# W-Ted/F3D-Gaus

Hardware: AMD Instinct MI355X
Metric: rendered views/sec at 256x256 (N Gaussians, K cams) (higher is better)
Workload: dtype f32; 1 GPU; C2: 1 image/GPU, 196608 Gaussians (sigma0=0.01), 120-view orbit @256x256, GOF forward raster only; timed region = render + 8-bit RGB frames copied to pinned host memory; compositing arithmetic: fast = error-free float32 pairs for the float64 island + hardware exp/rcp/rsq; every channel within 1e-4 of the oracle (RGB <= 3e-7), EXCEPT that the distortion channel (values 1e-7..1e-5 from cancelling fl; gaussians=196608, views=120, resolution=256, tile_cull=1, views_per_call=120, render_mode=fast, channels=all, parallelism=single GPU

## Files before the change

f3d-gaus_amd/csrc/f3dg_api.hip:

```cpp
#include "f3dg_common.h"

#include <stdio.h>
#include <string.h>
#include <time.h>
#include <mutex>
#include <vector>

namespace {

thread_local char g_last_error[512] = "";

size_t align_up(size_t x, size_t a) { return (x + a - 1) / a * a; }

__global__ void init_header_kernel(F3dgHeader* hdr, unsigned capacity, unsigned alpha_fast = 0, unsigned save_aux = 0)
{
    if (threadIdx.x < 64) {
        unsigned* w = reinterpret_cast<unsigned*>(hdr);
        w[threadIdx.x] = 0;
    }
    __syncthreads();
    if (threadIdx.x == 0) { hdr->capacity = capacity; hdr->alpha_fast = alpha_fast; hdr->save_aux = save_aux; }
}

__global__ void fill_background_kernel(int V, size_t HW, const float* __restrict__ bg, int bg_per_view,
// ... 175 lines not shown
    }
    g_prof.bwd.clear();
    if (h_calls) *h_calls = (int)g_prof.calls.size();
    g_prof.calls.clear();
    if (h_stage_ms) {
        for (int i = 0; i < ST_COUNT; i++) h_stage_ms[i] = sum[i];
        for (int i = 0; i < BW_COUNT; i++) h_stage_ms[ST_COUNT + i] = bsum[i];
    }
    return F3DG_OK;
}

int f3dg_set_hip_error(hipError_t e, const char* where)
{
    snprintf(g_last_error, sizeof g_last_error, "%s: %s", where, hipGetErrorString(e));
    return F3DG_ERR_HIP;
}

extern "C" const char* f3dg_version(void) { return "f3dg-hip gfx950 0.2.0"; }
extern "C" const char* f3dg_last_error(void) { return g_last_error; }

int f3dg_sort_passes(int V, int T);

F3dgLayout f3dg_layout(int P, int W, int H, int V, long long cap)
{
    F3dgLayout L;
    memset(&L, 0, sizeof L);
    const size_t VP = (size_t)V * (size_t)(P > 0 ? P : 1);
    const size_t HW = (size_t)W * H;
    const size_t T = (size_t)((W + F3DG_TILE - 1) / F3DG_TILE) * ((H + F3DG_TILE - 1) / F3DG_TILE);
    const size_t C = (size_t)(cap > 0 ? cap : 1);
    L.sort_blocks = (unsigned)((C + F3DG_SORT_CHUNK - 1) / F3DG_SORT_CHUNK);
    const size_t scan_a = (VP + F3DG_SCAN_CHUNK - 1) / F3DG_SCAN_CHUNK;
    const size_t gsort_blocks = (size_t)V * (((size_t)(P > 0 ? P : 1) + F3DG_SORT_CHUNK - 1) / F3DG_SORT_CHUNK);
    const size_t tile_blocks = (size_t)L.sort_blocks + (size_t)V;
    const size_t hist_blocks = gsort_blocks > tile_blocks ? gsort_blocks : tile_blocks;
    const size_t scan_b = ((size_t)256 * hist_blocks + F3DG_SCAN_CHUNK - 1) / F3DG_SCAN_CHUNK;
    L.scan_tmp_elems = (unsigned)((scan_a > scan_b ? scan_a : scan_b) + 1);

    size_t off = 0;
    auto take = [&](size_t bytes) { size_t o = off; off = align_up(off + bytes, 256); return o; };
    L.header = take(sizeof(F3dgHeader));
    L.rec = take(VP * sizeof(F3dgRec));
    L.means2D = take(VP * sizeof(float2));
    L.bbox = take(VP * sizeof(float4));
    L.cull = take(VP * sizeof(float4));
    L.depths = take(VP * sizeof(float));
    L.conic = take(VP * sizeof(float4));
    L.radii = take(VP * sizeof(int));
    L.tiles = take(VP * sizeof(unsigned));
    L.offsets = take(VP * sizeof(unsigned));
    L.clamped = take(VP);
    L.rects = take(VP * sizeof(uint2));
    L.gsort = take(4 * VP * sizeof(unsigned));
    L.scan_tmp = take((size_t)L.scan_tmp_elems * sizeof(unsigned));
    L.keys[0] = take(C * 8);
    L.keys[1] = take(C * 4);
    L.vals[0] = take(C * 4);
    L.vals[1] = take(C * 4);
    L.segtab_minmax = (unsigned)((size_t)2 * (V + 1) + (size_t)8 * (V / 8 + 2));
    L.segtab = take(((size_t)L.segtab_minmax + (size_t)2 * V + 2 * gsort_blocks) * sizeof(unsigned));
    L.hist = take((size_t)256 * hist_blocks * sizeof(unsigned));
    L.ranges = take((size_t)V * T * sizeof(uint2));
    L.final_T = take((size_t)V * 4 * HW * sizeof(float));
    L.n_contrib = take((size_t)V * 2 * HW * sizeof(unsigned));
    L.bwd_acc = take(VP * 16 * sizeof(double));
    L.small_cap = f3dg_small_shape(P, W, H, V) ? (unsigned)F3DG_SMALL_CAP : 0u;
    L.small_boxes = take(L.small_cap ? (size_t)V * ((P + 63) / 64) * sizeof(uint2) : 0);
    L.small_cnt = take((size_t)V * T * sizeof(unsigned));
// ... 446 lines not shown
```

f3d-gaus_amd/csrc/f3dg_binning.hip:

```cpp
#include "f3dg_common.h"

namespace {

typedef unsigned long long u64;
typedef unsigned int u32;

__global__ void __launch_bounds__(F3DG_BLOCK)
scan_reduce_kernel(const u32* __restrict__ in, u64 n, u32* __restrict__ block_sums)
{
    __shared__ u32 wsum[F3DG_BLOCK / 64];
    const u64 base = (u64)blockIdx.x * F3DG_SCAN_CHUNK;
    u32 s = 0;
#pragma unroll
    for (int i = 0; i < F3DG_SCAN_ITEMS; i++) {
        const u64 k = base + (u64)i * F3DG_BLOCK + threadIdx.x;
        if (k < n) s += in[k];
    }
#pragma unroll
    for (int off = 32; off > 0; off >>= 1) s += __shfl_down(s, off, 64);
    if ((threadIdx.x & 63) == 0) wsum[threadIdx.x >> 6] = s;
    __syncthreads();
    if (threadIdx.x == 0) block_sums[blockIdx.x] = wsum[0] + wsum[1] + wsum[2] + wsum[3];
}

// ... 140 lines not shown
                const u32 key = (u32)w[q];
                atomicAdd(&hw[digit(key)], 1u);
                if (MINMAX && key != 0xFFFFFFFFu) { kmin = key < kmin ? key : kmin; kmax = key > kmax ? key : kmax; }
            }
        }
    }
    __shared__ u32 wmm[2][F3DG_BLOCK / 64];
    if (MINMAX) {
#pragma unroll
        for (int off = 32; off > 0; off >>= 1) {
            const u32 a = __shfl_down(kmin, off, 64), b = __shfl_down(kmax, off, 64);
            kmin = a < kmin ? a : kmin; kmax = b > kmax ? b : kmax;
        }
        if ((threadIdx.x & 63) == 0) { wmm[0][threadIdx.x >> 6] = kmin; wmm[1][threadIdx.x >> 6] = kmax; }
    }
    __syncthreads();
    if (MINMAX && threadIdx.x == 0) {
        u32 a = wmm[0][0], b = wmm[1][0];
#pragma unroll
        for (int w = 1; w < F3DG_BLOCK / 64; w++) { a = wmm[0][w] < a ? wmm[0][w] : a; b = wmm[1][w] > b ? wmm[1][w] : b; }
        minmax[0] = a; minmax[1] = b;
    }
    hist[ck.obase + (u64)threadIdx.x * ck.cps + ck.c] = h[0][threadIdx.x] + h[1][threadIdx.x] + h[2][threadIdx.x] + h[3][threadIdx.x];
}

struct ScatterShared {
    u32 cnt[F3DG_BLOCK / 64][256];
    u32 lbase[256];
    u32 gdelta[256];
    u32 wtot[F3DG_BLOCK / 64];
    u32 sval[F3DG_SORT_CHUNK];
};

template <typename K, bool IOTA, typename DIGIT>
__device__ __forceinline__ void scatter_chunk(const K* __restrict__ keys_in, const u32* __restrict__ vals_in, K* __restrict__ keys_out,
                                              u32* __restrict__ vals_out, const SegChunk& ck, const DIGIT digit,
                                              const u32* __restrict__ offsets , ScatterShared& sh, K* skey)
{
    const u32 n = ck.n;
    const u64 block_base = (u64)ck.c * F3DG_SORT_CHUNK;
    const u32 in_block = (u32)((n - block_base) < (u64)F3DG_SORT_CHUNK ? (n - block_base) : (u64)F3DG_SORT_CHUNK);
    const int lane = threadIdx.x & 63, wave = threadIdx.x >> 6;
#pragma unroll
    for (int w = 0; w < F3DG_BLOCK / 64; w++) sh.cnt[w][threadIdx.x] = 0;
    __syncthreads();

    const u64 wave_base = block_base + (u64)wave * (64 * F3DG_SORT_ITEMS);
    u32 key[F3DG_SORT_ITEMS];
    u32 val[F3DG_SORT_ITEMS];
    u32 rank[F3DG_SORT_ITEMS];
    const u64 lane_lt = ((u64)1 << lane) - 1;
#pragma unroll
    for (int r = 0; r < F3DG_SORT_ITEMS; r++) {
        const u64 i = wave_base + (u64)r * 64 + lane;
        const bool valid = i < n;
        key[r] = valid ? (u32)keys_in[ck.seg_base + i] : 0u;
        val[r] = IOTA ? (u32)i : (valid ? vals_in[ck.seg_base + i] : 0u);
    }
#pragma unroll
    for (int r = 0; r < F3DG_SORT_ITEMS; r++) {
        const u64 i = wave_base + (u64)r * 64 + lane;
        const bool valid = i < n;
        const u32 d = digit(key[r]);
        u64 diff = 0;
#pragma unroll
        for (int b = 0; b < 8; b++) {
            const u32 own = (u32)((int)(d << (31 - b)) >> 31);
            const u64 bal = __ballot(own != 0u);
            diff |= bal ^ (((u64)own << 32) | own);
        }
        const u64 same = __ballot(valid) & ~diff;
        const u32 below = (u32)__popcll(same & lane_lt);
        const u32 prev = sh.cnt[wave][d];
        rank[r] = prev + below;
        __builtin_amdgcn_wave_barrier();
        if (valid && below == 0) sh.cnt[wave][d] = prev + (u32)__popcll(same);
        __builtin_amdgcn_wave_barrier();
    }
    __syncthreads();
    {
        const u32 d = threadIdx.x;
        const u32 c0 = sh.cnt[0][d], c1 = sh.cnt[1][d], c2 = sh.cnt[2][d], c3 = sh.cnt[3][d];
        const u32 tot = c0 + c1 + c2 + c3;
        u32 x = tot;
#pragma unroll
        for (int off = 1; off < 64; off <<= 1) {
            const u32 y = __shfl_up(x, off, 64);
            if (lane >= off) x += y;
        }
        if (lane == 63) sh.wtot[wave] = x;
        __syncthreads();
        u32 excl = x - tot;
        for (int w = 0; w < wave; w++) excl += sh.wtot[w];
        sh.lbase[d] = excl;
        sh.gdelta[d] = offsets[ck.obase + (u64)d * ck.cps + ck.c] - excl;
        sh.cnt[0][d] = excl;
        sh.cnt[1][d] = excl + c0;
        sh.cnt[2][d] = excl + c0 + c1;
        sh.cnt[3][d] = excl + c0 + c1 + c2;
    }
    __syncthreads();
#pragma unroll
    for (int r = 0; r < F3DG_SORT_ITEMS; r++) {
        const u64 i = wave_base + (u64)r * 64 + lane;
        if (i < n) {
            const u32 d = digit(key[r]);
            const u32 slot = sh.cnt[wave][d] + rank[r];
            skey[slot] = (K)key[r];
            sh.sval[slot] = val[r];
        }
    }
    __syncthreads();
    for (u32 slot = threadIdx.x; slot < in_block; slot += F3DG_BLOCK) {
        const K k = skey[slot];
        const u32 d = digit((u32)k);
        const u32 pos = sh.gdelta[d] + slot;
        if (keys_out) keys_out[pos] = k;
        vals_out[pos] = sh.sval[slot];
    }
}

__device__ __forceinline__ SegChunk fixed_chunk(u32 seg_len, u32 cps)
{
    u32 seg, c;
    f3dg_xcd_map(blockIdx.x, gridDim.x / cps, cps, seg, c);
    SegChunk ck;
    ck.seg_base = (u64)seg * seg_len; ck.obase = (u64)seg * 256u * cps; ck.n = seg_len; ck.cps = cps; ck.c = c; ck.seg = seg;
    return ck;
}

__device__ __forceinline__ bool gsort_compact(const u32* __restrict__ minmax, u32 view, u32& kbase)
{
    const u32 kmin = minmax[2 * view], kmax = minmax[2 * view + 1];
    kbase = kmin & 0xFFFF0000u;
    return kmin <= kmax && ((kmax - kbase) >> 24) == 0u;
}

template <int PASS>
__global__ void __launch_bounds__(F3DG_BLOCK)
gsort_hist_kernel(const u32* __restrict__ keys, u32 seg_len, u32 cps, u32* __restrict__ hist, const u32* __restrict__ minmax,
                  u32* __restrict__ chunk_minmax)
{
    __shared__ u32 h[F3DG_BLOCK / 64][256];
    const SegChunk ck = fixed_chunk(seg_len, cps);
    if constexpr (PASS == 0) {
        hist_chunk<u32, ShiftDigit>(keys, ck, ShiftDigit{0}, hist, h);
    } else if constexpr (PASS == 1) {
        hist_chunk<u32, ShiftDigit, true>(keys, ck, ShiftDigit{8}, hist, h, chunk_minmax + 2 * ((size_t)ck.seg * cps + ck.c));
    } else {
        u32 kbase;
        const bool compact = gsort_compact(minmax, ck.seg, kbase);
        if (!compact) {
// ... 49 lines not shown
        kmin = a < kmin ? a : kmin; kmax = b > kmax ? b : kmax;
    }
#pragma unroll
    for (int off = 32; off > 0; off >>= 1) {
        const u32 a = __shfl_down(kmin, off, 64), b = __shfl_down(kmax, off, 64);
        kmin = a < kmin ? a : kmin; kmax = b > kmax ? b : kmax;
    }
    if (threadIdx.x == 0) { minmax[2 * blockIdx.x] = kmin; minmax[2 * blockIdx.x + 1] = kmax; }
}

template <int PASS>
__global__ void __launch_bounds__(F3DG_BLOCK)
gsort_scatter_kernel(const u32* __restrict__ keys_in, const u32* __restrict__ vals_in, u32* __restrict__ keys_out,
                     u32* __restrict__ vals_out, u32 seg_len, u32 cps, const u32* __restrict__ offsets, const u32* __restrict__ minmax)
{
    __shared__ ScatterShared sh;
    __shared__ u32 skey[F3DG_SORT_CHUNK];
    const SegChunk ck = fixed_chunk(seg_len, cps);
    if constexpr (PASS == 0) {
        scatter_chunk<u32, true, ShiftDigit>(keys_in, vals_in, keys_out, vals_out, ck, ShiftDigit{0}, offsets, sh, skey);
    } else if constexpr (PASS == 1) {
        scatter_chunk<u32, false, ShiftDigit>(keys_in, vals_in, keys_out, vals_out, ck, ShiftDigit{8}, offsets, sh, skey);
    } else {
        u32 kbase;
        const bool compact = gsort_compact(minmax, ck.seg, kbase);
        if (!compact)
            scatter_chunk<u32, false, ShiftDigit>(keys_in, vals_in, PASS == 3 ? (u32*)nullptr : keys_out, vals_out, ck, ShiftDigit{8 * PASS}, offsets, sh, skey);
        else if constexpr (PASS == 2)
            scatter_chunk<u32, false, CompactDigit>(keys_in, vals_in, (u32*)nullptr, vals_out, ck, CompactDigit{kbase}, offsets, sh, skey);
    }
}

__global__ void __launch_bounds__(512)
view_segments_kernel(int V, int P, const u32* __restrict__ offsets_sorted, const F3dgHeader* __restrict__ hdr, u32* __restrict__ vstart,
                     u32* __restrict__ bglob, u32* __restrict__ xprefix, u32 xstride)
{
    __shared__ u32 carry;
    __shared__ u32 wtot[8];
    const u32 lane = threadIdx.x & 63u, wave = threadIdx.x >> 6;
    const bool dead = hdr->overflow != 0;
    auto start_of = [&](u32 v) -> u32 {
        const u64 i = (u64)v * (u64)P;
        return (dead || i == 0) ? 0u : offsets_sorted[i - 1];
    };
    auto chunks_of = [&](u32 v) -> u32 {
        const u32 n = start_of(v + 1) - start_of(v);
        return (n + F3DG_SORT_CHUNK - 1) / F3DG_SORT_CHUNK;
    };
    if (threadIdx.x == 0) carry = 0;
    __syncthreads();
    for (u32 v0 = 0; v0 < (u32)V; v0 += 512) {
        const u32 v = v0 + threadIdx.x;
        const u32 c = v < (u32)V ? chunks_of(v) : 0u;
        u32 x = c;
#pragma unroll
        for (int off = 1; off < 64; off <<= 1) {
            const u32 y = __shfl_up(x, off, 64);
            if (lane >= (u32)off) x += y;
        }
        if (lane == 63) wtot[wave] = x;
        __syncthreads();
        u32 woff = carry;
        for (u32 w = 0; w < wave; w++) woff += wtot[w];
        if (v < (u32)V) { vstart[v] = start_of(v); bglob[v] = woff + x - c; }
        __syncthreads();
        if (threadIdx.x == 511) carry = woff + x;
        __syncthreads();
    }
    if (threadIdx.x == 0) { vstart[V] = start_of((u32)V); bglob[V] = carry; }
    const u32 nk = ((u32)V > wave) ? ((u32)V - wave + 7u) / 8u : 0u;
    u32 run = 0;
    for (u32 k0 = 0; k0 < nk; k0 += 64) {
        const u32 k = k0 + lane;
        const u32 c = k < nk ? chunks_of(wave + 8u * k) : 0u;
        u32 x = c;
#pragma unroll
        for (int off = 1; off < 64; off <<= 1) {
            const u32 y = __shfl_up(x, off, 64);
            if (lane >= (u32)off) x += y;
        }
        if (k < nk) xprefix[wave * xstride + k] = run + x - c;
        run += __shfl(x, 63, 64);
    }
    if (lane == 0) xprefix[wave * xstride + nk] = run;
}

__global__ void __launch_bounds__(F3DG_BLOCK)
ranges_from_offsets_kernel(u32 V, u32 T, int tile_bits, const u32* __restrict__ bglob, const u32* __restrict__ offsets,
                           const F3dgHeader* __restrict__ hdr, uint2* __restrict__ ranges)
{
    const u32 i = blockIdx.x * F3DG_BLOCK + threadIdx.x;
    if (i >= V * T) return;
    const u32 v = i / T, t = i % T;
    const u32 b0 = bglob[v], cpv = bglob[v + 1] - b0;
    uint2 r = make_uint2(0u, 0u);
    if (cpv != 0u && !hdr->overflow) {
        const u32 d = ((v << tile_bits) | t) & 255u;
        const u32 lo = offsets[256ull * b0 + (u64)d * cpv], hi = offsets[256ull * b0 + (u64)(d + 1u) * cpv];
        if (hi > lo) r = make_uint2(lo, hi);
    }
    ranges[i] = r;
}

__device__ __forceinline__ bool var_chunk(const SegTable& st, u32 f, u32& k, SegChunk& ck)
{
    const u32 x = blockIdx.x & 7u;
    const u32* xp = st.xprefix + x * st.xstride;
    const u32 nk = (st.V > x) ? (st.V - x + 7u) / 8u : 0u;
    while (k < nk && f >= xp[k + 1]) k++;
    if (k >= nk) return false;
    const u32 v = x + 8u * k;
    const u32 s0 = st.vstart[v], b0 = st.bglob[v];
    ck.seg_base = s0; ck.n = st.vstart[v + 1] - s0; ck.cps = st.bglob[v + 1] - b0; ck.obase = 256ull * b0; ck.c = f - xp[k];
    return true;
}

template <typename K>
__global__ void __launch_bounds__(F3DG_BLOCK)
radix2_hist_var_kernel(const K* __restrict__ keys, SegTable st, int shift, u32 mask, u32* __restrict__ hist)
{
    __shared__ u32 h[F3DG_BLOCK / 64][256];
    u32 k = 0;
    SegChunk ck;
    for (u32 f = blockIdx.x >> 3; var_chunk(st, f, k, ck); f += gridDim.x >> 3)
        hist_chunk<K, ShiftDigit>(keys, ck, ShiftDigit{shift, mask}, hist, h);
}

template <typename K>
__global__ void __launch_bounds__(F3DG_BLOCK)
radix2_scatter_var_kernel(const K* __restrict__ keys_in, const u32* __restrict__ vals_in, K* __restrict__ keys_out,
                          u32* __restrict__ vals_out, SegTable st, int shift, u32 mask, const u32* __restrict__ offsets)
{
    __shared__ ScatterShared sh;
    __shared__ K skey[F3DG_SORT_CHUNK];
    u32 k = 0;
    SegChunk ck;
    for (u32 f = blockIdx.x >> 3; var_chunk(st, f, k, ck); f += gridDim.x >> 3) {
        scatter_chunk<K, false, ShiftDigit>(keys_in, vals_in, keys_out, vals_out, ck, ShiftDigit{shift, mask}, offsets, sh, skey);
        __syncthreads();
    }
}

__global__ void __launch_bounds__(F3DG_BLOCK)
gsort_gather_rects_kernel(int P, u32* __restrict__ gv0, u32* __restrict__ gv1, const u32* __restrict__ minmax,
                          const uint2* __restrict__ rects, u32* __restrict__ tiles_sorted, u32* __restrict__ rx)
{
    constexpr int ITEMS = 4;
    unsigned view, chunk;
    const unsigned cpv = (unsigned)((P + F3DG_BLOCK * ITEMS - 1) / (F3DG_BLOCK * ITEMS));
    f3dg_xcd_map(blockIdx.x, gridDim.x / cpv, cpv, view, chunk);
    const size_t vb = (size_t)view * P;
    u32 kbase;
    const bool pass2 = gsort_compact(minmax, view, kbase);
    const u32* perm = pass2 ? gv1 : gv0;
    u32* ry = pass2 ? gv0 : gv1;
    const int k0 = (int)(chunk * F3DG_BLOCK * ITEMS + threadIdx.x);
    u32 id[ITEMS];
    uint2 r[ITEMS];
#pragma unroll
    for (int i = 0; i < ITEMS; i++) { const int k = k0 + i * F3DG_BLOCK; id[i] = k < P ? perm[vb + k] : 0u; }
#pragma unroll
    for (int i = 0; i < ITEMS; i++) { const int k = k0 + i * F3DG_BLOCK; r[i] = k < P ? rects[vb + id[i]] : make_uint2(0u, 0u); }
#pragma unroll
    for (int i = 0; i < ITEMS; i++) {
        const int k = k0 + i * F3DG_BLOCK;
        if (k < P) {
            tiles_sorted[vb + k] = (((r[i].x >> 16) & F3DG_RECT_COORD) - (r[i].x & F3DG_RECT_COORD)) *
                                   (((r[i].y >> 16) & F3DG_RECT_COORD) - (r[i].y & F3DG_RECT_COORD));
            rx[vb + k] = r[i].x;
            ry[vb + k] = r[i].y;
        }
    }
}

#define F3DG_DUP_CAP 3072
template <typename G>
__global__ void __launch_bounds__(F3DG_BLOCK)
duplicate_sorted_kernel(int P, int tile_bits, int grid_x, const u32* __restrict__ gv0, const u32* __restrict__ gv1,
                        const u32* __restrict__ minmax, const u32* __restrict__ rx,
                        const u32* __restrict__ offsets_sorted,
                        const F3dgHeader* __restrict__ hdr, G* __restrict__ kgrp, u32* __restrict__ vals)
{
    __shared__ G sk[F3DG_DUP_CAP];
    __shared__ u32 sv[F3DG_DUP_CAP];
    if (hdr->overflow) return;
    const int k = blockIdx.x * F3DG_BLOCK + threadIdx.x;
    const int v = blockIdx.y;
    u32 kbase;
    const bool pass2 = gsort_compact(minmax, (u32)v, kbase);
    const u32* perm = pass2 ? gv1 : gv0;
    const u32* ry = pass2 ? gv0 : gv1;
    const size_t first = (size_t)v * P + (size_t)blockIdx.x * F3DG_BLOCK;
    const int in_block = min(F3DG_BLOCK, P - (int)(blockIdx.x * F3DG_BLOCK));
    const u32 base = first == 0 ? 0u : offsets_sorted[first - 1];
    const u32 n = offsets_sorted[first + in_block - 1] - base;
    u32 off0 = 0, cnt = 0, x = 0, y = 0, g = 0;
    if (k < P) {
        const size_t pos = (size_t)v * P + k;
        x = rx[pos]; y = ry[pos];
        const u32 rminx = x & F3DG_RECT_COORD, rmaxx = (x >> 16) & F3DG_RECT_COORD, rminy = y & F3DG_RECT_COORD, rmaxy = (y >> 16) & F3DG_RECT_COORD;
        if (rmaxx > rminx && rmaxy > rminy) {
            g = perm[pos];
            off0 = ((pos == 0) ? 0 : offsets_sorted[pos - 1]) - base;
            cnt = (rmaxx - rminx) * (rmaxy - rminy);
        }
    }
    const u32 rminx = x & F3DG_RECT_COORD, rmaxx = (x >> 16) & F3DG_RECT_COORD, rminy = y & F3DG_RECT_COORD, rmaxy = (y >> 16) & F3DG_RECT_COORD;
    const u32 view_base = (u32)v << tile_bits;
    auto halves = [](u32 t, u32 tmin, u32 tmax, u32 word) -> u32 {
        u32 m = 3u;
        if (t == tmin && (word & F3DG_RECT_SKIP_LO)) m &= ~1u;
        if (t + 1u == tmax && (word & F3DG_RECT_SKIP_HI)) m &= ~2u;
        return m;
    };
    for (u32 wb = 0; wb < n; wb += (u32)F3DG_DUP_CAP) {
        const u32 lo = off0 > wb ? off0 : wb;
        const u32 hi = off0 + cnt < wb + (u32)F3DG_DUP_CAP ? off0 + cnt : wb + (u32)F3DG_DUP_CAP;
        if (lo < hi) {
            const u32 w = rmaxx - rminx, j0 = lo - off0;
            u32 ty = rminy + j0 / w, tx = rminx + j0 % w;
            u32 my = halves(ty, rminy, rmaxy, y);
            for (u32 j = lo; j < hi; j++) {
                const u32 mx = halves(tx, rminx, rmaxx, x);
                sk[j - wb] = (G)(view_base | (ty * (u32)grid_x + tx));
                sv[j - wb] = g | ((((my & 1u) ? mx : 0u) | ((my & 2u) ? mx << 2 : 0u)) << F3DG_ID_BITS);
                if (++tx == rmaxx) { tx = rminx; ty++; my = halves(ty, rminy, rmaxy, y); }
            }
        }
        __syncthreads();
        const u32 in_win = n - wb < (u32)F3DG_DUP_CAP ? n - wb : (u32)F3DG_DUP_CAP;
        for (u32 i = threadIdx.x; i < in_win; i += F3DG_BLOCK) {
            kgrp[base + wb + i] = sk[i];
            vals[base + wb + i] = sv[i];
        }
        __syncthreads();
    }
}

__global__ void __launch_bounds__(F3DG_BLOCK)
export_keys_kernel(u32 nseg, int P, int tile_bits, int T, const uint2* __restrict__ ranges, const F3dgHeader* __restrict__ hdr,
                   const u32* __restrict__ point_list, const float* __restrict__ depths, u64* __restrict__ keys_out)
{
    if (hdr->overflow) return;
    for (u32 seg = blockIdx.x; seg < nseg; seg += gridDim.x) {
        const uint2 r = ranges[seg];
        const u32 view = seg / (u32)T, tile = seg % (u32)T;
        const u64 hi = (u64)((view << tile_bits) | tile) << 32;
        for (u32 i = r.x + threadIdx.x; i < r.y; i += F3DG_BLOCK)
            keys_out[i] = hi | (u64)__float_as_uint(depths[(size_t)view * P + (point_list[i] & F3DG_ID_MASK)]);
    }
}

template <typename G>
__global__ void __launch_bounds__(F3DG_BLOCK)
group_bounds_kernel(const G* __restrict__ kgrp, const F3dgHeader* __restrict__ hdr, int tile_bits, int T, u32* __restrict__ ranges)
{
    const u32 L = hdr->overflow ? 0u : hdr->num_rendered;
    const u32 tmask = (1u << tile_bits) - 1u;
    for (u64 base = ((u64)blockIdx.x * F3DG_BLOCK + threadIdx.x) * 8u; base < L; base += (u64)gridDim.x * F3DG_BLOCK * 8u) {
        G v[8];
        if (base + 8 <= L) {
            typedef G __attribute__((ext_vector_type(8))) G8;
            const G8 w = *reinterpret_cast<const G8*>(kgrp + base);
#pragma unroll
            for (int i = 0; i < 8; i++) v[i] = w[i];
        } else {
#pragma unroll
// ... 29 lines not shown
                               unsigned* tmp, unsigned tmp_elems, int exclusive, F3dgHeader* hdr_total)
{
    if (n == 0) return F3DG_OK;
    const unsigned nblocks = (unsigned)((n + F3DG_SCAN_CHUNK - 1) / F3DG_SCAN_CHUNK);
    if (nblocks > tmp_elems) return F3DG_ERR_WORKSPACE;
    F3DG_KLAUNCH(scan_reduce_kernel, dim3(nblocks), dim3(F3DG_BLOCK), 0, s, in, (u64)n, tmp);
    F3DG_KLAUNCH(scan_blocksums_kernel, dim3(1), dim3(1024), 0, s, tmp, nblocks, hdr_total);
    F3DG_KLAUNCH(scan_apply_kernel, dim3(nblocks), dim3(F3DG_BLOCK), 0, s, in, out, (u64)n, tmp, exclusive);
    F3DG_HIP_CHECK(hipGetLastError());
    return F3DG_OK;
}

int f3dg_tile_bits(int T) { return bits_for((unsigned long long)T); }


int f3dg_sort_passes(int V, int T)
{
    (void)V;
    const int bits = f3dg_tile_bits(T);
    return bits == 0 ? 0 : (bits + 7) / 8;
}

template <typename G>
static int binning_tail(hipStream_t s, int V, int P, int grid_x, int T, int tile_bits, const F3dgLayout& L, char* ws, F3dgHeader* hdr)
{
    int rc = F3DG_OK;
    const size_t VP = (size_t)V * P;
    u32* scan_tmp = reinterpret_cast<u32*>(ws + L.scan_tmp);
    u32* hist = reinterpret_cast<u32*>(ws + L.hist);
    u32* gk[2] = { reinterpret_cast<u32*>(ws + L.gsort), reinterpret_cast<u32*>(ws + L.gsort) + VP };
    u32* gv[2] = { reinterpret_cast<u32*>(ws + L.gsort) + 2 * VP, reinterpret_cast<u32*>(ws + L.gsort) + 3 * VP };
    G* kgrp[2] = { reinterpret_cast<G*>(ws + L.keys[0]), reinterpret_cast<G*>(ws + L.keys[1]) };
    u32* vals[2] = { reinterpret_cast<u32*>(ws + L.vals[0]), reinterpret_cast<u32*>(ws + L.vals[1]) };
    const dim3 pgrid((P + F3DG_BLOCK - 1) / F3DG_BLOCK, V);

    const u32 cps = (u32)((P + F3DG_SORT_CHUNK - 1) / F3DG_SORT_CHUNK);
    const u32 gblocks = (u32)V * cps;
    u32* minmax = reinterpret_cast<u32*>(ws + L.segtab) + L.segtab_minmax;
    u32* chunk_minmax = minmax + 2 * (size_t)V;
    const bool view_scan = cps <= 64;
#define F3DG_GSORT_PASS(PASS, IN, OUT)                                                                                                     \
    F3DG_KLAUNCH((gsort_hist_kernel<PASS>), dim3(gblocks), dim3(F3DG_BLOCK), 0, s, gk[IN], (u32)P, cps, hist, minmax, chunk_minmax); \
    if (view_scan)                                                                                                                         \
        F3DG_KLAUNCH(gsort_scan_kernel, dim3(V), dim3(1024), 0, s, 256u * cps, (u32)P, hist);                                       \
    else {                                                                                                                                 \
        rc = f3dg_launch_scan_inclusive(s, hist, hist, (unsigned long long)256 * gblocks, scan_tmp, L.scan_tmp_elems, 1, nullptr);        \
        if (rc != F3DG_OK) return rc;                                                                                                      \
    }                                                                                                                                      \
    F3DG_KLAUNCH((gsort_scatter_kernel<PASS>), dim3(gblocks), dim3(F3DG_BLOCK), 0, s, gk[IN], gv[IN], gk[OUT], gv[OUT], (u32)P, cps, hist, minmax)
    F3DG_GSORT_PASS(0, 0, 1);
    F3DG_GSORT_PASS(1, 1, 0);
    F3DG_KLAUNCH(gsort_range_kernel, dim3(V), dim3(64), 0, s, cps, chunk_minmax, minmax);
    F3DG_GSORT_PASS(2, 0, 1);
    F3DG_GSORT_PASS(3, 1, 0);
#undef F3DG_GSORT_PASS
    u32* offsets_sorted = gk[1];
    u32* rx = gk[0];

    F3DG_KLAUNCH(gsort_gather_rects_kernel, dim3((unsigned)V * (unsigned)((P + 4 * F3DG_BLOCK - 1) / (4 * F3DG_BLOCK))), dim3(F3DG_BLOCK), 0, s, P, gv[0], gv[1], minmax,
                           reinterpret_cast<const uint2*>(ws + L.rects), offsets_sorted, rx);
    rc = f3dg_launch_scan_inclusive(s, offsets_sorted, offsets_sorted, (unsigned long long)VP, scan_tmp, L.scan_tmp_elems, 0, hdr);
    if (rc != F3DG_OK) return rc;
    const int passes = f3dg_sort_passes(V, T);
    int src = passes & 1;
    F3DG_KLAUNCH((duplicate_sorted_kernel<G>), pgrid, dim3(F3DG_BLOCK), 0, s, P, tile_bits, grid_x, gv[0], gv[1], minmax, rx, offsets_sorted, hdr,
                       kgrp[src], vals[src]);

    if (passes > 0) {
        SegTable st;
        u32* segtab = reinterpret_cast<u32*>(ws + L.segtab);
        const u32 xstride = (u32)V / 8u + 2u;
        st.vstart = segtab; st.bglob = segtab + (V + 1); st.xprefix = segtab + 2 * (V + 1); st.xstride = xstride; st.V = (u32)V;
        F3DG_KLAUNCH(view_segments_kernel, dim3(1), dim3(512), 0, s, V, P, offsets_sorted, hdr, segtab, segtab + (V + 1),
                           segtab + 2 * (V + 1), xstride);
        const size_t nbmax = (size_t)L.sort_blocks + (size_t)V;
        const u32 per_xcd = (u32)((nbmax + 7) / 8 < 160 ? (nbmax + 7) / 8 : 160);
        const u32 per_xcd_h = (u32)((nbmax + 7) / 8 < 512 ? (nbmax + 7) / 8 : 512);
        const int split = passes == 2 ? (tile_bits + 1) / 2 : 8;
        for (int p = 0; p < passes; p++) {
            const int shift = split * p;
            const u32 mask = passes == 2 ? (1u << (p == 0 ? split : tile_bits - split)) - 1u : 255u;
            F3DG_HIP_CHECK(hipMemsetAsync(hist, 0, sizeof(u32) * 256 * nbmax, s));
            F3DG_KLAUNCH((radix2_hist_var_kernel<G>), dim3(8 * per_xcd_h), dim3(F3DG_BLOCK), 0, s, kgrp[src], st, shift, mask, hist);
            rc = f3dg_launch_scan_inclusive(s, hist, hist, (unsigned long long)256 * nbmax, scan_tmp, L.scan_tmp_elems, 1, nullptr);
            if (rc != F3DG_OK) return rc;
            F3DG_KLAUNCH((radix2_scatter_var_kernel<G>), dim3(8 * per_xcd), dim3(F3DG_BLOCK), 0, s, kgrp[src], vals[src],
                               passes == 1 ? (G*)nullptr : kgrp[src ^ 1], vals[src ^ 1], st, shift, mask, hist);
            src ^= 1;
        }
        if (passes == 1) {
            const u32 nseg = (u32)V * (u32)T;
            F3DG_KLAUNCH(ranges_from_offsets_kernel, dim3((nseg + F3DG_BLOCK - 1) / F3DG_BLOCK), dim3(F3DG_BLOCK), 0, s, (u32)V, (u32)T, tile_bits,
                               segtab + (V + 1), hist, hdr, reinterpret_cast<uint2*>(ws + L.ranges));
            F3DG_HIP_CHECK(hipGetLastError());
            return F3DG_OK;
        }
    }
    F3DG_HIP_CHECK(hipMemsetAsync(ws + L.ranges, 0, sizeof(uint2) * (size_t)V * T, s));
    F3DG_KLAUNCH((group_bounds_kernel<G>), dim3(2048), dim3(F3DG_BLOCK), 0, s, kgrp[0], hdr, tile_bits, T, reinterpret_cast<u32*>(ws + L.ranges));
    F3DG_HIP_CHECK(hipGetLastError());
    return F3DG_OK;
}

int f3dg_launch_binning(hipStream_t s, int V, int P, int W, int H, const F3dgLayout& L, char* ws, int export_offsets)
{
    const int grid_x = (W + F3DG_TILE - 1) / F3DG_TILE, grid_y = (H + F3DG_TILE - 1) / F3DG_TILE;
    const int T = grid_x * grid_y;
    const int tile_bits = f3dg_tile_bits(T);
    F3dgHeader* hdr = reinterpret_cast<F3dgHeader*>(ws + L.header);

    int rc = F3DG_OK;
    if (export_offsets) {
        rc = f3dg_launch_scan_inclusive(s, reinterpret_cast<const u32*>(ws + L.tiles), reinterpret_cast<u32*>(ws + L.offsets),
                                        (unsigned long long)V * P, reinterpret_cast<u32*>(ws + L.scan_tmp), L.scan_tmp_elems, 0, nullptr);
        if (rc != F3DG_OK) return rc;
    }
    const bool small = (((unsigned long long)(V > 0 ? V - 1 : 0) << tile_bits) | ((1ull << tile_bits) - 1ull)) <= 0xFFFFull;
    rc = small ? binning_tail<unsigned short>(s, V, P, grid_x, T, tile_bits, L, ws, hdr)
               : binning_tail<u32>(s, V, P, grid_x, T, tile_bits, L, ws, hdr);
    if (rc != F3DG_OK) return rc;
    F3DG_HIP_CHECK(hipGetLastError());
    return F3DG_OK;
}

int f3dg_launch_export_keys(hipStream_t s, int V, int P, int W, int H, const F3dgLayout& L, char* ws)
{
    const int grid_x = (W + F3DG_TILE - 1) / F3DG_TILE, grid_y = (H + F3DG_TILE - 1) / F3DG_TILE;
    const int T = grid_x * grid_y;
    const u32 nseg = (u32)V * (u32)T;
// ... 9 lines not shown
```

f3d-gaus_amd/csrc/f3dg_common.h:

```cpp
#pragma once
#include <hip/hip_runtime.h>
#include <stddef.h>
#include <stdint.h>

#include "../../include/f3dg.h"

#define F3DG_BLOCK 256
#define F3DG_REC_FLOATS 16
#define F3DG_NEAR_PLANE 0.2
#define F3DG_FAR_PLANE 100.0
#define F3DG_SORT_ITEMS 16
#define F3DG_SORT_CHUNK (F3DG_BLOCK * F3DG_SORT_ITEMS)
#define F3DG_SCAN_ITEMS 16
#define F3DG_SCAN_CHUNK (F3DG_BLOCK * F3DG_SCAN_ITEMS)

#define F3DG_ID_BITS 28
#define F3DG_ID_MASK 0x0FFFFFFFu
#define F3DG_RECT_COORD 0x7FFFu
#define F3DG_RECT_SKIP_LO 0x8000u
#define F3DG_RECT_SKIP_HI 0x80000000u

__device__ __forceinline__ void f3dg_xcd_map(unsigned b, unsigned V, unsigned U, unsigned& view, unsigned& unit)
{
    const unsigned full = (V & ~7u) * U;
    if (b < full) {
        const unsigned slot = b >> 3;
        view = (slot / U) * 8u + (b & 7u);
        unit = slot % U;
    } else {
        const unsigned r = b - full;
        view = (V & ~7u) + r / U;
        unit = r % U;
    }
}

struct F3dgHeader {
    unsigned int num_rendered;
    unsigned int overflow;
    unsigned int capacity;
    unsigned int bwd_stale;
    unsigned int reserved1[2];
    unsigned int alpha_fast;
    unsigned int save_aux;
    unsigned long long bwd_pairs;
    unsigned int small_path;
// ... 172 lines not shown
```

Measured before the change: 30360 views/s.

## Fuse tile duplication with first radix pass via per-chunk digit histograms

Replaces the gather-rects + global offset scan + duplicate kernel + first radix hist/scatter sequence with a count kernel that builds per-chunk digit histograms of tile keys directly from rects, one scan over those histograms, and a scatter kernel that expands instances into shared memory and writes them already ordered by the low digit. This removes one full write and read of the duplicated key/value arrays plus one radix pass. View segment boundaries and ranges are now derived from the histogram offsets. The scatter kernel carries more shared memory and recomputes rect areas and prefix sums per window.

```diff
diff --git a/f3d-gaus_amd/csrc/f3dg_api.hip b/f3d-gaus_amd/csrc/f3dg_api.hip
--- a/f3d-gaus_amd/csrc/f3dg_api.hip
+++ b/f3d-gaus_amd/csrc/f3dg_api.hip
@@ -231,8 +231,9 @@
     L.sort_blocks = (unsigned)((C + F3DG_SORT_CHUNK - 1) / F3DG_SORT_CHUNK);
     const size_t scan_a = (VP + F3DG_SCAN_CHUNK - 1) / F3DG_SCAN_CHUNK;
     const size_t gsort_blocks = (size_t)V * (((size_t)(P > 0 ? P : 1) + F3DG_SORT_CHUNK - 1) / F3DG_SORT_CHUNK);
+    const size_t bin_blocks = (size_t)V * (((size_t)(P > 0 ? P : 1) + F3DG_BIN_CHUNK - 1) / F3DG_BIN_CHUNK);
     const size_t tile_blocks = (size_t)L.sort_blocks + (size_t)V;
-    const size_t hist_blocks = gsort_blocks > tile_blocks ? gsort_blocks : tile_blocks;
+    const size_t hist_blocks = bin_blocks > tile_blocks ? bin_blocks : tile_blocks;
     const size_t scan_b = ((size_t)256 * hist_blocks + F3DG_SCAN_CHUNK - 1) / F3DG_SCAN_CHUNK;
     L.scan_tmp_elems = (unsigned)((scan_a > scan_b ? scan_a : scan_b) + 1);
 
diff --git a/f3d-gaus_amd/csrc/f3dg_binning.hip b/f3d-gaus_amd/csrc/f3dg_binning.hip
--- a/f3d-gaus_amd/csrc/f3dg_binning.hip
+++ b/f3d-gaus_amd/csrc/f3dg_binning.hip
@@ -196,35 +196,29 @@
     u32 sval[F3DG_SORT_CHUNK];
 };
 
-template <typename K, bool IOTA, typename DIGIT>
-__device__ __forceinline__ void scatter_chunk(const K* __restrict__ keys_in, const u32* __restrict__ vals_in, K* __restrict__ keys_out,
-                                              u32* __restrict__ vals_out, const SegChunk& ck, const DIGIT digit,
-                                              const u32* __restrict__ offsets , ScatterShared& sh, K* skey)
-{
-    const u32 n = ck.n;
-    const u64 block_base = (u64)ck.c * F3DG_SORT_CHUNK;
-    const u32 in_block = (u32)((n - block_base) < (u64)F3DG_SORT_CHUNK ? (n - block_base) : (u64)F3DG_SORT_CHUNK);
+template <typename K, typename DIGIT, typename LOAD, typename BASE>
+__device__ __forceinline__ void scatter_block(const u32 in_block, LOAD load, BASE base, K* __restrict__ keys_out, u32* __restrict__ vals_out,
+                                              const DIGIT digit, ScatterShared& sh, K* skey)
+{
     const int lane = threadIdx.x & 63, wave = threadIdx.x >> 6;
 #pragma unroll
     for (int w = 0; w < F3DG_BLOCK / 64; w++) sh.cnt[w][threadIdx.x] = 0;
     __syncthreads();
 
-    const u64 wave_base = block_base + (u64)wave * (64 * F3DG_SORT_ITEMS);
+    const u32 wave_base = (u32)wave * (64 * F3DG_SORT_ITEMS);
     u32 key[F3DG_SORT_ITEMS];
     u32 val[F3DG_SORT_ITEMS];
     u32 rank[F3DG_SORT_ITEMS];
     const u64 lane_lt = ((u64)1 << lane) - 1;
 #pragma unroll
     for (int r = 0; r < F3DG_SORT_ITEMS; r++) {
-        const u64 i = wave_base + (u64)r * 64 + lane;
-        const bool valid = i < n;
-        key[r] = valid ? (u32)keys_in[ck.seg_base + i] : 0u;
-        val[r] = IOTA ? (u32)i : (valid ? vals_in[ck.seg_base + i] : 0u);
+        const u32 j = wave_base + (u32)r * 64 + lane;
+        load(j, j < in_block, key[r], val[r]);
     }
 #pragma unroll
     for (int r = 0; r < F3DG_SORT_ITEMS; r++) {
-        const u64 i = wave_base + (u64)r * 64 + lane;
-        const bool valid = i < n;
+        const u32 j = wave_base + (u32)r * 64 + lane;
+        const bool valid = j < in_block;
         const u32 d = digit(key[r]);
         u64 diff = 0;
 #pragma unroll
@@ -257,7 +251,7 @@
         u32 excl = x - tot;
         for (int w = 0; w < wave; w++) excl += sh.wtot[w];
         sh.lbase[d] = excl;
-        sh.gdelta[d] = offsets[ck.obase + (u64)d * ck.cps + ck.c] - excl;
+        sh.gdelta[d] = base(d, tot) - excl;
         sh.cnt[0][d] = excl;
         sh.cnt[1][d] = excl + c0;
         sh.cnt[2][d] = excl + c0 + c1;
@@ -266,8 +260,8 @@
     __syncthreads();
 #pragma unroll
     for (int r = 0; r < F3DG_SORT_ITEMS; r++) {
-        const u64 i = wave_base + (u64)r * 64 + lane;
-        if (i < n) {
+        const u32 j = wave_base + (u32)r * 64 + lane;
+        if (j < in_block) {
             const u32 d = digit(key[r]);
             const u32 slot = sh.cnt[wave][d] + rank[r];
             skey[slot] = (K)key[r];
@@ -282,6 +276,23 @@
         if (keys_out) keys_out[pos] = k;
         vals_out[pos] = sh.sval[slot];
     }
+}
+
+template <typename K, bool IOTA, typename DIGIT>
+__device__ __forceinline__ void scatter_chunk(const K* __restrict__ keys_in, const u32* __restrict__ vals_in, K* __restrict__ keys_out,
+                                              u32* __restrict__ vals_out, const SegChunk& ck, const DIGIT digit,
+                                              const u32* __restrict__ offsets , ScatterShared& sh, K* skey)
+{
+    const u64 block_base = (u64)ck.c * F3DG_SORT_CHUNK;
+    const u32 in_block = (u32)((ck.n - block_base) < (u64)F3DG_SORT_CHUNK ? (ck.n - block_base) : (u64)F3DG_SORT_CHUNK);
+    const u64 first = ck.seg_base + block_base;
+    scatter_block<K, DIGIT>(in_block,
+        [&](u32 j, bool valid, u32& key, u32& val) {
+            key = valid ? (u32)keys_in[first + j] : 0u;
+            val = IOTA ? (u32)block_base + j : (valid ? vals_in[first + j] : 0u);
+        },
+        [&](u32 d, u32) { return offsets[ck.obase + (u64)d * ck.cps + ck.c]; },
+        keys_out, vals_out, digit, sh, skey);
 }
 
 __device__ __forceinline__ SegChunk fixed_chunk(u32 seg_len, u32 cps)
@@ -397,7 +408,7 @@
 }
 
 __global__ void __launch_bounds__(512)
-view_segments_kernel(int V, int P, const u32* __restrict__ offsets_sorted, const F3dgHeader* __restrict__ hdr, u32* __restrict__ vstart,
+view_segments_kernel(int V, u32 cpv, const u32* __restrict__ offsets, const F3dgHeader* __restrict__ hdr, u32* __restrict__ vstart,
                      u32* __restrict__ bglob, u32* __restrict__ xprefix, u32 xstride)
 {
     __shared__ u32 carry;
@@ -405,8 +416,7 @@
     const u32 lane = threadIdx.x & 63u, wave = threadIdx.x >> 6;
     const bool dead = hdr->overflow != 0;
     auto start_of = [&](u32 v) -> u32 {
-        const u64 i = (u64)v * (u64)P;
-        return (dead || i == 0) ? 0u : offsets_sorted[i - 1];
+        return dead ? 0u : (v == (u32)V ? hdr->num_rendered : offsets[256ull * cpv * v]);
     };
     auto chunks_of = [&](u32 v) -> u32 {
         const u32 n = start_of(v + 1) - start_of(v);
@@ -451,17 +461,17 @@
 }
 
 __global__ void __launch_bounds__(F3DG_BLOCK)
-ranges_from_offsets_kernel(u32 V, u32 T, int tile_bits, const u32* __restrict__ bglob, const u32* __restrict__ offsets,
+ranges_from_offsets_kernel(u32 V, u32 T, int tile_bits, u32 cpv, const u32* __restrict__ offsets,
                            const F3dgHeader* __restrict__ hdr, uint2* __restrict__ ranges)
 {
     const u32 i = blockIdx.x * F3DG_BLOCK + threadIdx.x;
     if (i >= V * T) return;
     const u32 v = i / T, t = i % T;
-    const u32 b0 = bglob[v], cpv = bglob[v + 1] - b0;
     uint2 r = make_uint2(0u, 0u);
-    if (cpv != 0u && !hdr->overflow) {
+    if (!hdr->overflow) {
         const u32 d = ((v << tile_bits) | t) & 255u;
-        const u32 lo = offsets[256ull * b0 + (u64)d * cpv], hi = offsets[256ull * b0 + (u64)(d + 1u) * cpv];
+        const u64 e = (256ull * v + d) * cpv, end = 256ull * V * cpv;
+        const u32 lo = offsets[e], hi = e + cpv < end ? offsets[e + cpv] : hdr->num_rendered;
         if (hi > lo) r = make_uint2(lo, hi);
     }
     ranges[i] = r;
@@ -506,98 +516,152 @@
     }
 }
 
-__global__ void __launch_bounds__(F3DG_BLOCK)
-gsort_gather_rects_kernel(int P, u32* __restrict__ gv0, u32* __restrict__ gv1, const u32* __restrict__ minmax,
-                          const uint2* __restrict__ rects, u32* __restrict__ tiles_sorted, u32* __restrict__ rx)
-{
-    constexpr int ITEMS = 4;
-    unsigned view, chunk;
-    const unsigned cpv = (unsigned)((P + F3DG_BLOCK * ITEMS - 1) / (F3DG_BLOCK * ITEMS));
-    f3dg_xcd_map(blockIdx.x, gridDim.x / cpv, cpv, view, chunk);
-    const size_t vb = (size_t)view * P;
-    u32 kbase;
-    const bool pass2 = gsort_compact(minmax, view, kbase);
-    const u32* perm = pass2 ? gv1 : gv0;
-    u32* ry = pass2 ? gv0 : gv1;
-    const int k0 = (int)(chunk * F3DG_BLOCK * ITEMS + threadIdx.x);
-    u32 id[ITEMS];
-    uint2 r[ITEMS];
-#pragma unroll
-    for (int i = 0; i < ITEMS; i++) { const int k = k0 + i * F3DG_BLOCK; id[i] = k < P ? perm[vb + k] : 0u; }
-#pragma unroll
-    for (int i = 0; i < ITEMS; i++) { const int k = k0 + i * F3DG_BLOCK; r[i] = k < P ? rects[vb + id[i]] : make_uint2(0u, 0u); }
-#pragma unroll
-    for (int i = 0; i < ITEMS; i++) {
-        const int k = k0 + i * F3DG_BLOCK;
-        if (k < P) {
-            tiles_sorted[vb + k] = (((r[i].x >> 16) & F3DG_RECT_COORD) - (r[i].x & F3DG_RECT_COORD)) *
-                                   (((r[i].y >> 16) & F3DG_RECT_COORD) - (r[i].y & F3DG_RECT_COORD));
-            rx[vb + k] = r[i].x;
-            ry[vb + k] = r[i].y;
-        }
-    }
-}
-
-#define F3DG_DUP_CAP 3072
-template <typename G>
-__global__ void __launch_bounds__(F3DG_BLOCK)
-duplicate_sorted_kernel(int P, int tile_bits, int grid_x, const u32* __restrict__ gv0, const u32* __restrict__ gv1,
-                        const u32* __restrict__ minmax, const u32* __restrict__ rx,
-                        const u32* __restrict__ offsets_sorted,
-                        const F3dgHeader* __restrict__ hdr, G* __restrict__ kgrp, u32* __restrict__ vals)
-{
-    __shared__ G sk[F3DG_DUP_CAP];
-    __shared__ u32 sv[F3DG_DUP_CAP];
-    if (hdr->overflow) return;
-    const int k = blockIdx.x * F3DG_BLOCK + threadIdx.x;
-    const int v = blockIdx.y;
-    u32 kbase;
-    const bool pass2 = gsort_compact(minmax, (u32)v, kbase);
-    const u32* perm = pass2 ? gv1 : gv0;
-    const u32* ry = pass2 ? gv0 : gv1;
-    const size_t first = (size_t)v * P + (size_t)blockIdx.x * F3DG_BLOCK;
-    const int in_block = min(F3DG_BLOCK, P - (int)(blockIdx.x * F3DG_BLOCK));
-    const u32 base = first == 0 ? 0u : offsets_sorted[first - 1];
-    const u32 n = offsets_sorted[first + in_block - 1] - base;
-    u32 off0 = 0, cnt = 0, x = 0, y = 0, g = 0;
-    if (k < P) {
-        const size_t pos = (size_t)v * P + k;
-        x = rx[pos]; y = ry[pos];
-        const u32 rminx = x & F3DG_RECT_COORD, rmaxx = (x >> 16) & F3DG_RECT_COORD, rminy = y & F3DG_RECT_COORD, rmaxy = (y >> 16) & F3DG_RECT_COORD;
-        if (rmaxx > rminx && rmaxy > rminy) {
-            g = perm[pos];
-            off0 = ((pos == 0) ? 0 : offsets_sorted[pos - 1]) - base;
-            cnt = (rmaxx - rminx) * (rmaxy - rminy);
-        }
-    }
+
+__device__ __forceinline__ u32 rect_area(u32 x, u32 y)
+{
     const u32 rminx = x & F3DG_RECT_COORD, rmaxx = (x >> 16) & F3DG_RECT_COORD, rminy = y & F3DG_RECT_COORD, rmaxy = (y >> 16) & F3DG_RECT_COORD;
-    const u32 view_base = (u32)v << tile_bits;
+    return (rmaxx > rminx && rmaxy > rminy) ? (rmaxx - rminx) * (rmaxy - rminy) : 0u;
+}
+
+template <typename F>
+__device__ __forceinline__ void rect_instances(u32 x, u32 y, u32 grid_x, u32 j0, u32 j1, F f)
+{
+    const u32 rminx = x & F3DG_RECT_COORD, rmaxx = (x >> 16) & F3DG_RECT_COORD, rminy = y & F3DG_RECT_COORD, rmaxy = (y >> 16) & F3DG_RECT_COORD;
     auto halves = [](u32 t, u32 tmin, u32 tmax, u32 word) -> u32 {
         u32 m = 3u;
         if (t == tmin && (word & F3DG_RECT_SKIP_LO)) m &= ~1u;
         if (t + 1u == tmax && (word & F3DG_RECT_SKIP_HI)) m &= ~2u;
         return m;
     };
-    for (u32 wb = 0; wb < n; wb += (u32)F3DG_DUP_CAP) {
-        const u32 lo = off0 > wb ? off0 : wb;
-        const u32 hi = off0 + cnt < wb + (u32)F3DG_DUP_CAP ? off0 + cnt : wb + (u32)F3DG_DUP_CAP;
-        if (lo < hi) {
-            const u32 w = rmaxx - rminx, j0 = lo - off0;
-            u32 ty = rminy + j0 / w, tx = rminx + j0 % w;
-            u32 my = halves(ty, rminy, rmaxy, y);
-            for (u32 j = lo; j < hi; j++) {
-                const u32 mx = halves(tx, rminx, rmaxx, x);
-                sk[j - wb] = (G)(view_base | (ty * (u32)grid_x + tx));
-                sv[j - wb] = g | ((((my & 1u) ? mx : 0u) | ((my & 2u) ? mx << 2 : 0u)) << F3DG_ID_BITS);
-                if (++tx == rmaxx) { tx = rminx; ty++; my = halves(ty, rminy, rmaxy, y); }
+    u32 ty = rminy, tx = rminx;
+    if (j0 != 0u) { const u32 w = rmaxx - rminx; ty += j0 / w; tx += j0 % w; }
+    u32 my = halves(ty, rminy, rmaxy, y);
+    for (u32 j = j0; j < j1; j++) {
+        const u32 mx = halves(tx, rminx, rmaxx, x);
+        f(j, ty * grid_x + tx, ((my & 1u) ? mx : 0u) | ((my & 2u) ? mx << 2 : 0u));
+        if (++tx == rmaxx) { tx = rminx; ty++; my = halves(ty, rminy, rmaxy, y); }
+    }
+}
+
+struct BinChunk {
+    u32 view, chunk;
+    const u32* perm;
+    u32* ry;
+};
+__device__ __forceinline__ BinChunk bin_chunk(u32 cpv, u32* gv0, u32* gv1, const u32* __restrict__ minmax)
+{
+    BinChunk bc;
+    f3dg_xcd_map(blockIdx.x, gridDim.x / cpv, cpv, bc.view, bc.chunk);
+    u32 kbase;
+    const bool pass2 = gsort_compact(minmax, bc.view, kbase);
+    bc.perm = pass2 ? gv1 : gv0;
+    bc.ry = pass2 ? gv0 : gv1;
+    return bc;
+}
+
+__global__ void __launch_bounds__(F3DG_BLOCK)
+bin_gather_count_kernel(int P, u32 cpv, int tile_bits, u32 grid_x, ShiftDigit digit, u32* __restrict__ gv0, u32* __restrict__ gv1,
+                        const u32* __restrict__ minmax, const uint2* __restrict__ rects, u32* __restrict__ rx, u32* __restrict__ hist)
+{
+    __shared__ u32 h[F3DG_BLOCK / 64][256];
+    const BinChunk bc = bin_chunk(cpv, gv0, gv1, minmax);
+    const size_t vb = (size_t)bc.view * P;
+    const u32 k0 = bc.chunk * F3DG_BIN_CHUNK + threadIdx.x;
+    u32 id[F3DG_BIN_ITEMS];
+    uint2 r[F3DG_BIN_ITEMS];
+#pragma unroll
+    for (int i = 0; i < F3DG_BIN_ITEMS; i++) { const u32 k = k0 + i * F3DG_BLOCK; id[i] = k < (u32)P ? bc.perm[vb + k] : 0u; }
+#pragma unroll
+    for (int i = 0; i < F3DG_BIN_ITEMS; i++) { const u32 k = k0 + i * F3DG_BLOCK; r[i] = k < (u32)P ? rects[vb + id[i]] : make_uint2(0u, 0u); }
+#pragma unroll
+    for (int w = 0; w < F3DG_BLOCK / 64; w++) h[w][threadIdx.x] = 0;
+    __syncthreads();
+    u32* hw = h[threadIdx.x >> 6];
+    const u32 view_base = bc.view << tile_bits;
+#pragma unroll
+    for (int i = 0; i < F3DG_BIN_ITEMS; i++) {
+        const u32 k = k0 + i * F3DG_BLOCK;
+        if (k < (u32)P) {
+            rx[vb + k] = r[i].x;
+            bc.ry[vb + k] = r[i].y;
+            rect_instances(r[i].x, r[i].y, grid_x, 0u, rect_area(r[i].x, r[i].y),
+                           [&](u32, u32 tile, u32) { atomicAdd(&hw[digit(view_base | tile)], 1u); });
+        }
+    }
+    __syncthreads();
+    hist[((size_t)bc.view * 256u + threadIdx.x) * cpv + bc.chunk] = h[0][threadIdx.x] + h[1][threadIdx.x] + h[2][threadIdx.x] + h[3][threadIdx.x];
+}
+
+template <typename G>
+__global__ void __launch_bounds__(F3DG_BLOCK)
+bin_scatter_kernel(int P, u32 cpv, int tile_bits, u32 grid_x, ShiftDigit digit, u32* gv0, u32* gv1, const u32* __restrict__ minmax,
+                   const u32* __restrict__ rx, const u32* __restrict__ offsets ,
+                   const F3dgHeader* __restrict__ hdr, G* __restrict__ kgrp_out ,
+                   u32* __restrict__ vals_out)
+{
+    __shared__ ScatterShared sh;
+    __shared__ G skey[F3DG_SORT_CHUNK];
+    __shared__ u32 rtot[F3DG_BIN_ITEMS][F3DG_BLOCK / 64];
+    if (hdr->overflow) return;
+    const BinChunk bc = bin_chunk(cpv, gv0, gv1, minmax);
+    const size_t vb = (size_t)bc.view * P;
+    const u32 k0 = bc.chunk * F3DG_BIN_CHUNK + threadIdx.x;
+    const u32 lane = threadIdx.x & 63u, wave = threadIdx.x >> 6;
+    u32 off0[F3DG_BIN_ITEMS];
+#pragma unroll
+    for (int i = 0; i < F3DG_BIN_ITEMS; i++) {
+        const u32 k = k0 + i * F3DG_BLOCK;
+        const u32 cnt = k < (u32)P ? rect_area(rx[vb + k], bc.ry[vb + k]) : 0u;
+        u32 s = cnt;
+#pragma unroll
+        for (int off = 1; off < 64; off <<= 1) {
+            const u32 t = __shfl_up(s, off, 64);
+            if (lane >= (u32)off) s += t;
+        }
+        if (lane == 63u) rtot[i][wave] = s;
+        off0[i] = s - cnt;
+    }
+    __syncthreads();
+    u32 n = 0;
+#pragma unroll
+    for (int i = 0; i < F3DG_BIN_ITEMS; i++)
+#pragma unroll
+        for (int w = 0; w < F3DG_BLOCK / 64; w++) {
+            const u32 t = rtot[i][w];
+            if ((u32)w < wave) off0[i] += t;
+#pragma unroll
+            for (int i2 = i + 1; i2 < F3DG_BIN_ITEMS; i2++) off0[i2] += t;
+            n += t;
+        }
+    if (n == 0u) return;
+    const u32 nwin = (n + F3DG_SORT_CHUNK - 1) / F3DG_SORT_CHUNK, win = (n + nwin - 1) / nwin;
+    const u32 view_base = bc.view << tile_bits;
+    u32 gpos = offsets[((size_t)bc.view * 256u + threadIdx.x) * cpv + bc.chunk];
+    for (u32 wb = 0; wb < n; wb += win) {
+        const u32 in_win = n - wb < win ? n - wb : win;
+        u32 kw = k0;
+        asm volatile("" : "+v"(kw));
+#pragma unroll
+        for (int i = 0; i < F3DG_BIN_ITEMS; i++) {
+            const u32 k = kw + i * F3DG_BLOCK;
+            if (k >= (u32)P || off0[i] >= wb + in_win) continue;
+            const u32 x = rx[vb + k], y = bc.ry[vb + k];
+            const u32 end = off0[i] + rect_area(x, y);
+            const u32 lo = off0[i] > wb ? off0[i] : wb;
+            const u32 hi = end < wb + in_win ? end : wb + in_win;
+            if (lo < hi) {
+                const u32 g = bc.perm[vb + k];
+                const u32 at = off0[i] - wb;
+                rect_instances(x, y, grid_x, lo - off0[i], hi - off0[i], [&](u32 j, u32 tile, u32 qmask) {
+                    skey[at + j] = (G)(view_base | tile);
+                    sh.sval[at + j] = g | (qmask << F3DG_ID_BITS);
+                });
             }
         }
-        __syncthreads();
-        const u32 in_win = n - wb < (u32)F3DG_DUP_CAP ? n - wb : (u32)F3DG_DUP_CAP;
-        for (u32 i = threadIdx.x; i < in_win; i += F3DG_BLOCK) {
-            kgrp[base + wb + i] = sk[i];
-            vals[base + wb + i] = sv[i];
-        }
+        scatter_block<G, ShiftDigit>(in_win,
+            [&](u32 j, bool valid, u32& key, u32& val) { key = valid ? (u32)skey[j] : 0u; val = valid ? sh.sval[j] : 0u; },
+            [&](u32, u32 tot) { const u32 p = gpos; gpos += tot; return p; },
+            kgrp_out, vals_out, digit, sh, skey);
         __syncthreads();
     }
 }
@@ -693,7 +757,6 @@
     u32* gv[2] = { reinterpret_cast<u32*>(ws + L.gsort) + 2 * VP, reinterpret_cast<u32*>(ws + L.gsort) + 3 * VP };
     G* kgrp[2] = { reinterpret_cast<G*>(ws + L.keys[0]), reinterpret_cast<G*>(ws + L.keys[1]) };
     u32* vals[2] = { reinterpret_cast<u32*>(ws + L.vals[0]), reinterpret_cast<u32*>(ws + L.vals[1]) };
-    const dim3 pgrid((P + F3DG_BLOCK - 1) / F3DG_BLOCK, V);
 
     const u32 cps = (u32)((P + F3DG_SORT_CHUNK - 1) / F3DG_SORT_CHUNK);
     const u32 gblocks = (u32)V * cps;
@@ -715,47 +778,44 @@
     F3DG_GSORT_PASS(2, 0, 1);
     F3DG_GSORT_PASS(3, 1, 0);
 #undef F3DG_GSORT_PASS
-    u32* offsets_sorted = gk[1];
     u32* rx = gk[0];
 
-    F3DG_KLAUNCH(gsort_gather_rects_kernel, dim3((unsigned)V * (unsigned)((P + 4 * F3DG_BLOCK - 1) / (4 * F3DG_BLOCK))), dim3(F3DG_BLOCK), 0, s, P, gv[0], gv[1], minmax,
-                           reinterpret_cast<const uint2*>(ws + L.rects), offsets_sorted, rx);
-    rc = f3dg_launch_scan_inclusive(s, offsets_sorted, offsets_sorted, (unsigned long long)VP, scan_tmp, L.scan_tmp_elems, 0, hdr);
+    const int passes = f3dg_sort_passes(V, T);
+    const int split = passes == 2 ? (tile_bits + 1) / 2 : 8;
+    const u32 cpv = (u32)((P + F3DG_BIN_CHUNK - 1) / F3DG_BIN_CHUNK);
+    const ShiftDigit digit0{0, passes == 2 ? (1u << split) - 1u : 255u};
+    const int dst = passes == 2 ? 1 : 0;
+    F3DG_KLAUNCH(bin_gather_count_kernel, dim3((u32)V * cpv), dim3(F3DG_BLOCK), 0, s, P, cpv, tile_bits, (u32)grid_x, digit0, gv[0], gv[1], minmax,
+                       reinterpret_cast<const uint2*>(ws + L.rects), rx, hist);
+    rc = f3dg_launch_scan_inclusive(s, hist, hist, 256ull * V * cpv, scan_tmp, L.scan_tmp_elems, 1, hdr);
     if (rc != F3DG_OK) return rc;
-    const int passes = f3dg_sort_passes(V, T);
-    int src = passes & 1;
-    F3DG_KLAUNCH((duplicate_sorted_kernel<G>), pgrid, dim3(F3DG_BLOCK), 0, s, P, tile_bits, grid_x, gv[0], gv[1], minmax, rx, offsets_sorted, hdr,
-                       kgrp[src], vals[src]);
-
-    if (passes > 0) {
-        SegTable st;
-        u32* segtab = reinterpret_cast<u32*>(ws + L.segtab);
+    SegTable st;
+    u32* segtab = reinterpret_cast<u32*>(ws + L.segtab);
+    if (passes == 2) {
         const u32 xstride = (u32)V / 8u + 2u;
         st.vstart = segtab; st.bglob = segtab + (V + 1); st.xprefix = segtab + 2 * (V + 1); st.xstride = xstride; st.V = (u32)V;
-        F3DG_KLAUNCH(view_segments_kernel, dim3(1), dim3(512), 0, s, V, P, offsets_sorted, hdr, segtab, segtab + (V + 1),
-                           segtab + 2 * (V + 1), xstride);
+        F3DG_KLAUNCH(view_segments_kernel, dim3(1), dim3(512), 0, s, V, cpv, hist, hdr, segtab, segtab + (V + 1), segtab + 2 * (V + 1), xstride);
+    }
+    F3DG_KLAUNCH((bin_scatter_kernel<G>), dim3((u32)V * cpv), dim3(F3DG_BLOCK), 0, s, P, cpv, tile_bits, (u32)grid_x, digit0, gv[0], gv[1], minmax, rx,
+                       hist, hdr, passes == 2 ? kgrp[dst] : (G*)nullptr, vals[dst]);
+    if (passes < 2) {
+        const u32 nseg = (u32)V * (u32)T;
+        F3DG_KLAUNCH(ranges_from_offsets_kernel, dim3((nseg + F3DG_BLOCK - 1) / F3DG_BLOCK), dim3(F3DG_BLOCK), 0, s, (u32)V, (u32)T, tile_bits,
+                           cpv, hist, hdr, reinterpret_cast<uint2*>(ws + L.ranges));
+        F3DG_HIP_CHECK(hipGetLastError());
+        return F3DG_OK;
+    }
+
+    {
         const size_t nbmax = (size_t)L.sort_blocks + (size_t)V;
         const u32 per_xcd = (u32)((nbmax + 7) / 8 < 160 ? (nbmax + 7) / 8 : 160);
         const u32 per_xcd_h = (u32)((nbmax + 7) / 8 < 512 ? (nbmax + 7) / 8 : 512);
-        const int split = passes == 2 ? (tile_bits + 1) / 2 : 8;
-        for (int p = 0; p < passes; p++) {
-            const int shift = split * p;
-            const u32 mask = passes == 2 ? (1u << (p == 0 ? split : tile_bits - split)) - 1u : 255u;
-            F3DG_HIP_CHECK(hipMemsetAsync(hist, 0, sizeof(u32) * 256 * nbmax, s));
-            F3DG_KLAUNCH((radix2_hist_var_kernel<G>), dim3(8 * per_xcd_h), dim3(F3DG_BLOCK), 0, s, kgrp[src], st, shift, mask, hist);
-            rc = f3dg_launch_scan_inclusive(s, hist, hist, (unsigned long long)256 * nbmax, scan_tmp, L.scan_tmp_elems, 1, nullptr);
-            if (rc != F3DG_OK) return rc;
-            F3DG_KLAUNCH((radix2_scatter_var_kernel<G>), dim3(8 * per_xcd), dim3(F3DG_BLOCK), 0, s, kgrp[src], vals[src],
-                               passes == 1 ? (G*)nullptr : kgrp[src ^ 1], vals[src ^ 1], st, shift, mask, hist);
-            src ^= 1;
-        }
-        if (passes == 1) {
-            const u32 nseg = (u32)V * (u32)T;
-            F3DG_KLAUNCH(ranges_from_offsets_kernel, dim3((nseg + F3DG_BLOCK - 1) / F3DG_BLOCK), dim3(F3DG_BLOCK), 0, s, (u32)V, (u32)T, tile_bits,
-                               segtab + (V + 1), hist, hdr, reinterpret_cast<uint2*>(ws + L.ranges));
-            F3DG_HIP_CHECK(hipGetLastError());
-            return F3DG_OK;
-        }
+        const u32 mask = (1u << (tile_bits - split)) - 1u;
+        F3DG_HIP_CHECK(hipMemsetAsync(hist, 0, sizeof(u32) * 256 * nbmax, s));
+        F3DG_KLAUNCH((radix2_hist_var_kernel<G>), dim3(8 * per_xcd_h), dim3(F3DG_BLOCK), 0, s, kgrp[1], st, split, mask, hist);
+        rc = f3dg_launch_scan_inclusive(s, hist, hist, (unsigned long long)256 * nbmax, scan_tmp, L.scan_tmp_elems, 1, nullptr);
+        if (rc != F3DG_OK) return rc;
+        F3DG_KLAUNCH((radix2_scatter_var_kernel<G>), dim3(8 * per_xcd), dim3(F3DG_BLOCK), 0, s, kgrp[1], vals[1], kgrp[0], vals[0], st, split, mask, hist);
     }
     F3DG_HIP_CHECK(hipMemsetAsync(ws + L.ranges, 0, sizeof(uint2) * (size_t)V * T, s));
     F3DG_KLAUNCH((group_bounds_kernel<G>), dim3(2048), dim3(F3DG_BLOCK), 0, s, kgrp[0], hdr, tile_bits, T, reinterpret_cast<u32*>(ws + L.ranges));
diff --git a/f3d-gaus_amd/csrc/f3dg_common.h b/f3d-gaus_amd/csrc/f3dg_common.h
--- a/f3d-gaus_amd/csrc/f3dg_common.h
+++ b/f3d-gaus_amd/csrc/f3dg_common.h
@@ -11,6 +11,8 @@
 #define F3DG_FAR_PLANE 100.0
 #define F3DG_SORT_ITEMS 16
 #define F3DG_SORT_CHUNK (F3DG_BLOCK * F3DG_SORT_ITEMS)
+#define F3DG_BIN_ITEMS 4
+#define F3DG_BIN_CHUNK (F3DG_BLOCK * F3DG_BIN_ITEMS)
 #define F3DG_SCAN_ITEMS 16
 #define F3DG_SCAN_CHUNK (F3DG_BLOCK * F3DG_SCAN_ITEMS)
 
```

Result: no change. 30350 views/s (median of 4 runs) (-0.0%).
